# Ai00-X/ai00_server

Measured on AMD Instinct MI355X. Metric: decode tokens/sec (whole job), higher is better.
Workload: dtype u8->f16/f32acc; 1 GPU; RWKV-v6-3b int8 decode, batch=32/GPU, greedy, state+tokens resident in HBM; quant=int8, batch_per_gpu=32, parallelism=replicas x1 (no collective)

## Files before the change

### ai00_server_amd/build.py

```python
from __future__ import annotations

import os
import subprocess
import sys

HERE = os.path.dirname(os.path.abspath(__file__))
CSRC = os.path.join(HERE, "csrc")
LIB = os.path.join(HERE, "librwkv_hip.so")
SOURCES = ["rwkv_kernels.hip", "rwkv_engine.cpp", "tokenizer.cpp"]
DEPS = SOURCES + ["rwkv_kernels.h", "gemm_plan.h", "graph_cache.h", "gen_stop.h", "safetensors.hpp", "rwkv_abi.map", os.path.join("..", "..", "include", "rwkv_abi.h"),
               os.path.join("..", "..", "include", "rwkv_runtime.hpp"), os.path.join("..", "..", "include", "rwkv_scheduler.hpp"),
               os.path.join("..", "..", "include", "rwkv_router.hpp"),
               os.path.join("..", "..", "harness", "decode_loop.cpp"), os.path.join("..", "..", "harness", "serve_loop.cpp"),
               os.path.join("..", "..", "harness", "router_loop.cpp")]


def _hipcc() -> str:
    for c in (os.environ.get("HIPCC"), "/opt/rocm/bin/hipcc", "hipcc"):
        if c and (os.path.isabs(c) and os.path.exists(c) or not os.path.isabs(c)):
            return c
    return "hipcc"


STAMP = os.path.join(HERE, ".build_stamp")


def _sources_digest() -> str:
    import hashlib
    h = hashlib.sha256()
    for d in sorted(DEPS):
        with open(os.path.join(CSRC, d), "rb") as f:
            h.update(d.encode())
            h.update(f.read())
    return h.hexdigest()


def needs_build() -> bool:
    if not all(os.path.exists(p) for p in (LIB, HARNESS_BIN, SERVE_BIN, ROUTER_BIN, EMBED_BIN, STAMP)):
        return True
    return open(STAMP).read().strip() != _sources_digest()


KERNEL_PARTS = 6


def build(force: bool = False, verbose: bool = True) -> str:
    if not force and not needs_build():
        return LIB
    from concurrent.futures import ThreadPoolExecutor
    hipcc = _hipcc()
    jobs = []
    for src in SOURCES:
        stem = os.path.splitext(src)[0]
        base = [hipcc, "--offload-arch=gfx950", "-O3", "-std=c++17", "-fPIC"]
        if src.endswith(".cpp"):
            base += ["-x", "hip"]
        if src == "rwkv_kernels.hip":
            for k in range(KERNEL_PARTS):
                obj = os.path.join(CSRC, f"{stem}.p{k}.o")
                jobs.append((base + [f"-DRWKV_PART={k}", "-c", os.path.join(CSRC, src), "-o", obj], obj))
        else:
            obj = os.path.join(CSRC, stem + ".o")
            jobs.append((base + ["-c", os.path.join(CSRC, src), "-o", obj], obj))

    def run(job):
        if verbose:
            print("[build]", " ".join(job[0]), flush=True)
        subprocess.check_call(job[0])
        return job[1]

    with ThreadPoolExecutor(max_workers=min(len(jobs), os.cpu_count() or 4)) as ex:
        objs = list(ex.map(run, jobs))
    cmd = [hipcc, "--offload-arch=gfx950", "-shared", "-fPIC", "-Wl,--version-script=" + os.path.join(CSRC, "rwkv_abi.map"), "-o", LIB] + objs
    if verbose:
        print("[build]", " ".join(cmd), flush=True)
    subprocess.check_call(cmd)
    build_harness(verbose)
    with open(STAMP, "w") as f:
        f.write(_sources_digest())
    return LIB


HARNESS_SRC = os.path.join(HERE, "..", "harness", "decode_loop.cpp")
HARNESS_BIN = os.path.join(HERE, "..", "harness", "decode_loop")
SERVE_SRC = os.path.join(HERE, "..", "harness", "serve_loop.cpp")
SERVE_BIN = os.path.join(HERE, "..", "harness", "serve_loop")
ROUTER_SRC = os.path.join(HERE, "..", "harness", "router_loop.cpp")
ROUTER_BIN = os.path.join(HERE, "..", "harness", "router_loop")
EMBED_SRC = os.path.join(HERE, "..", "harness", "embed_job.cpp")
EMBED_BIN = os.path.join(HERE, "..", "harness", "embed_job")


def build_harness(verbose: bool = True) -> str:
    for src, exe in ((HARNESS_SRC, HARNESS_BIN), (SERVE_SRC, SERVE_BIN), (ROUTER_SRC, ROUTER_BIN), (EMBED_SRC, EMBED_BIN)):
        cmd = ["g++", "-O2", "-std=c++17", "-pthread", src, "-o", exe, "-L" + HERE, "-lrwkv_hip", "-Wl,-rpath," + HERE]
        if verbose:
            print("[build]", " ".join(cmd), flush=True)
        subprocess.check_call(cmd)
    return HARNESS_BIN


PROBE_DIR = os.path.join(HERE, "..", "tests", "cpp")
PROBE_SRC = os.path.join(PROBE_DIR, "gemm_probe.hip")
PROBE_BIN = os.path.join(PROBE_DIR, "gemm_probe")
PROBE_STAMP = os.path.join(PROBE_DIR, ".gemm_probe_stamp")


def compile_gemm_probe(obj: str) -> str:
    subprocess.check_call([_hipcc(), "--offload-arch=gfx950", "-O2", "-std=c++17", "-c", PROBE_SRC, "-o", obj])
    return obj


def build_gemm_probe(verbose: bool = True) -> str:
    import hashlib
    build(verbose=verbose)
    h = hashlib.sha256(_sources_digest().encode())
    for src in (PROBE_SRC, os.path.join(PROBE_DIR, "gemm_probe_plan.h")):
        with open(src, "rb") as f:
            h.update(f.read())
    if os.path.exists(PROBE_BIN) and os.path.exists(PROBE_STAMP) and open(PROBE_STAMP).read().strip() == h.hexdigest():
        return PROBE_BIN
    parts = [os.path.join(CSRC, f"rwkv_kernels.p{k}.o") for k in range(KERNEL_PARTS)]
    if not all(os.path.exists(p) for p in parts):
        build(force=True, verbose=verbose)
    obj = compile_gemm_probe(os.path.join(PROBE_DIR, "gemm_probe.o"))
    cmd = [_hipcc(), "--offload-arch=gfx950", obj] + parts + ["-o", PROBE_BIN]
    if verbose:
        print("[build]", " ".join(cmd), flush=True)
    subprocess.check_call(cmd)
    with open(PROBE_STAMP, "w") as f:
        f.write(h.hexdigest())
    return PROBE_BIN


if __name__ == "__main__":
    build(force="--force" in sys.argv)
    print(LIB)
```

### ai00_server_amd/csrc/rwkv_kernels.h

```cpp
#pragma once
#ifdef __HIP__
#include <hip/hip_runtime.h>
#else
typedef struct ihipStream_t *hipStream_t;
#ifndef __FLT16_MANT_DIG__
typedef unsigned short _Float16;
#endif
#endif
#include <stddef.h>
#include <stdint.h>

#include "gen_stop.h"

namespace rwkv {

enum WFmt : int { W_F16 = 0, W_INT8 = 1, W_NF4 = 2 };
enum Act : int { ACT_NONE = 0, ACT_TANH = 1, ACT_SIGMOID = 2, ACT_RELU2 = 3, ACT_SILU = 4, ACT_DECAY7 = 5 };
enum Post : int { POST_NONE = 0, POST_MUL = 1, POST_MIX = 2 };

struct Knobs {
    int no_ln_fuse = 0;
    int no_v6_fuse = 0;
    int no_tile = 0, tile_shape = -1;
    int no_dense = 0;
    int tile_ksplit = 1;
    int tile_xcd = -1;
    int promote = -1;
    int v6_ksp_max = 16;
    int v6_ksp_blocks = 160, v6_ksp_min_t = 192;
    static Knobs from_env();
};
const Knobs &knobs();
void use_knobs(const Knobs &k);

constexpr int TILE_ROWS = 16;
constexpr int KSTEP = 32;
constexpr int GEMM_MAX_WAVES = 10;
constexpr int GEMM_MAX_WAVES_K16 = 8;
constexpr int GEMM_MAXP = 8;
constexpr int INT8_BLOCK = 128;
constexpr int NF4_BLOCK = 64;

struct DMat {
    const void *data = nullptr;
    const void *scales = nullptr;
    int fmt = W_F16;
    int rows = 0;
    int K = 0;
    uint64_t bytes = 0;
};

struct RowMeta {
    const int *token;
    const int *slot;
    const int *prev;
    const int *last;
    int dense;
};

constexpr int LNP_MAX_T = 1;
constexpr int LNP_MAX_NP = 5;
struct LnProArgs {
    const float *x_in;
    float *x_out;
    const float *P;
    int np;
    long pstride;
    const float *lnw, *lnb;
    const float *sx;
    long sx_slot_stride;
    RowMeta rm;
    int mode;
    float *xx_out;
    int C;
};
struct ShiftCommit {
    const float *src;
    float *sx;
    long sx_slot_stride;
    RowMeta rm;
    int T, C;
};

struct GemmProb {
    const void *W;
    const void *S;
    const _Float16 *xhi;
    const _Float16 *xlo;
    int fmt, rows, K, ldx;
    int spb;
    int nw;
    int ksb;
    int Kb, nslice;
    int nblk_strip;
    int block_begin;
    int act, post;
    const float *bias;
    const float *m0, *m1;
    int ldm;
    float *out_f32;
    int ldo;
    long partial_stride;
    _Float16 *out_hi, *out_lo;
    int ldh;
};

struct GemmLaunch {
    GemmProb p[GEMM_MAXP];
    int nprob;
    int T;
    int threads;
    int lds_items;
    int single_shot;
    int tail;
    int total_blocks;
    int xcd_map;
    ShiftCommit commit;
};

size_t lnp_lds_bytes(int T, int C, bool hilo);
void launch_gemm(const GemmLaunch &L, bool hilo, hipStream_t s);
void launch_smallk(const GemmLaunch &L, bool hilo, hipStream_t s);
void launch_gemm_tile45(const GemmLaunch &L, int kind, int ntl, bool hilo, hipStream_t s);
void launch_gemm_tile(const GemmLaunch &L, int shape, bool hilo, hipStream_t s);

struct V6MixArgs {
    const void *W1;
    const void *W2[5];
    const _Float16 *zhi, *zlo;
    int ldz;
    const float *xx, *dx;
    const float *mu[5];
    _Float16 *ohi[5], *olo[5];
    int ldh, T, C, Dm;
    LnProArgs lnp;
    const float *mu_x;
    _Float16 *mg_hi = nullptr, *mg_lo = nullptr;
    float *mp = nullptr;
    int ksp = 1, ksp_min_t = 192, ksp_blocks = 160, ksp_max = 16;
};
bool v6_mix_supported(int T, int C, int Dm);
bool v6_mix_wide_supported(int T, int C, int Dm);
bool v6_mix_ln_supported(int T, int C, int Dm, bool hilo, int np);
int v6_mix_split(const V6MixArgs &a, bool hilo);
void launch_v6_mix(const V6MixArgs &a, bool hilo, hipStream_t s);


struct LnShiftArgs {
    const float *x_in;
    float *x_out;
    const float *P;
    int np;
    long pstride;
    const float *lnw, *lnb;
    float *sx;
    long sx_slot_stride;
    RowMeta rm;
    int mode;
    int nmix;
    const float *mu[6];
    _Float16 *ohi[6];
    _Float16 *olo[6];
    int ldh;
    float *xx_out, *dx_out;
    int C;
    int xcd_rows = 0;
};
void launch_ln_shift(const LnShiftArgs &a, int T, hipStream_t s);

struct EmbedArgs {
    const _Float16 *emb;
    const float *lnw, *lnb;
    const int *token;
    float *x;
    int C, V;
};
void launch_embed(const EmbedArgs &a, int T, hipStream_t s);

struct LnOutArgs {
    const float *x_in;
    const float *P;
    int np;
    long pstride;
    const float *lnw, *lnb;
    const int *out_rows;
    _Float16 *ohi, *olo;
    int ldh, C;
};
void launch_ln_out(const LnOutArgs &a, int n_out, hipStream_t s);

struct WkvArgs {
    int version;
    int H, C;
    int n_seq;
    const int *seq_slot;
    const int *seq_begin;
    const int *seq_len;
    int dense;
    float *state;
    long slot_stride;
    const float *r, *k, *v;
    const float *g;
    const float *wdec_or_decay;
    const float *u;
    const float *td;
    const _Float16 *D2;
    int Dd;
    const float *w7, *a7, *vg7;
    const float *k_k, *k_a, *r_k;
    float *v_first;
    int layer;
    const float *lnx_w, *lnx_b;
    _Float16 *yhi, *ylo;
    int ldh;
    int max_rows;
};
void launch_wkv(const WkvArgs &a, bool multi_row, hipStream_t s);

struct StatePackArgs {
    float *slab;
    float *sxa, *sxf;
    float *wkv;
    int L, C, H;
    int transposed;
    int to_slab;
    int layer_only;
};
void launch_state_pack(const StatePackArgs &a, hipStream_t s);

void launch_softmax(const float *in, float *out, int n_rows, int V, hipStream_t s);
void launch_score_rows(const float *logits, const unsigned *targets, float *out, int n_rows, int V, hipStream_t s);
struct SampleRow { float top_p; int top_k; float temperature; float uniform; int kind; float tau; };
void launch_logit_adjust(float *logits, int V, const int *rows, const int *toks, const float *vals, int n, hipStream_t s);
void launch_logit_mask(float *logits, int V, const int *rows, const unsigned char *allow, int n, hipStream_t s);
void launch_nucleus(const float *logits, int n_rows, int V, const SampleRow *sp, bool any_nucleus_typical, bool any_mirostat,
                    int *out_tok, float *out_prob, hipStream_t s);
constexpr unsigned GEN_ABSENT = 0xFFFFFFFFu;
constexpr int GEN_MAX_STOP = 8;
struct GenSlot {
    float top_p; int top_k; float temperature; float tau;
    int kind;
    float presence, frequency, decay;
    float miro_target, miro_rate;
    unsigned long long seed;
    unsigned stream, draws;
    int max_tokens, emitted, finish;
    int freeze_at;
    int has_bias, n_stop;
    unsigned stop[GEN_MAX_STOP];
// ... 52 lines not shown
```

### ai00_server_amd/csrc/rwkv_kernels.hip

```cpp
#include "gemm_plan.h"
#include <type_traits>
#include <cstdlib>
#include <algorithm>


#ifdef RWKV_PART
#define RWKV_PART_ON(k) (RWKV_PART == (k))
#else
#define RWKV_PART_ON(k) 1
#endif
#if defined(RWKV_TRACE) && defined(RWKV_PART)
#error "trace builds are single-part"
#endif

namespace rwkv {

typedef _Float16 f16x8 __attribute__((ext_vector_type(8)));
typedef _Float16 f16x4 __attribute__((ext_vector_type(4)));
typedef _Float16 f16x2 __attribute__((ext_vector_type(2)));
typedef float f32x4 __attribute__((ext_vector_type(4)));
typedef float f32x2 __attribute__((ext_vector_type(2)));
typedef unsigned int u32;
typedef unsigned int u32x4 __attribute__((ext_vector_type(4)));
typedef unsigned int u32x2 __attribute__((ext_vector_type(2)));

__device__ __forceinline__ float sigmoidf_(float x) { return 1.0f / (1.0f + expf(-x)); }

__device__ __forceinline__ float apply_act(int act, float v) {
    switch (act) {
        case ACT_TANH: return tanhf(v);
        case ACT_SIGMOID: return sigmoidf_(v);
        case ACT_RELU2: { float r = fmaxf(v, 0.0f); return r * r; }
        case ACT_SILU: return v * sigmoidf_(v);
        case ACT_DECAY7: return expf(-0.606531f * sigmoidf_(v));
        default: return v;
    }
}

__device__ __forceinline__ void apply_act4(int act, float (&v)[4]) {
    switch (act) {
        case ACT_NONE: break;
        case ACT_TANH: for (int r = 0; r < 4; ++r) v[r] = tanhf(v[r]); break;
        case ACT_SIGMOID: for (int r = 0; r < 4; ++r) v[r] = sigmoidf_(v[r]); break;
        case ACT_RELU2: for (int r = 0; r < 4; ++r) { const float q = fmaxf(v[r], 0.0f); v[r] = q * q; } break;
        case ACT_SILU: for (int r = 0; r < 4; ++r) v[r] = v[r] * sigmoidf_(v[r]); break;
        case ACT_DECAY7: for (int r = 0; r < 4; ++r) v[r] = expf(-0.606531f * sigmoidf_(v[r])); break;
        default: break;
    }
}
__device__ __forceinline__ void split_hilo(float v, _Float16 &hi, _Float16 &lo) {
    float c = fminf(fmaxf(v, -65504.0f), 65504.0f);
    hi = (_Float16)c;
    lo = (_Float16)(c - (float)hi);
}

__device__ __forceinline__ long opd_off(int t, int k, int ld) {
    return ((long)(t >> 4) * (ld >> 5) + (k >> 5)) * 512 + ((((k >> 3) & 3) << 4) + (t & 15)) * 8 + (k & 7);
}

__device__ __forceinline__ void store_operand4(_Float16 *__restrict__ hi, _Float16 *__restrict__ lo, long off, float4 o) {
    f16x4 h, l;
    _Float16 a, b;
    split_hilo(o.x, a, b); h[0] = a; l[0] = b;
    split_hilo(o.y, a, b); h[1] = a; l[1] = b;
    split_hilo(o.z, a, b); h[2] = a; l[2] = b;
    split_hilo(o.w, a, b); h[3] = a; l[3] = b;
    *(f16x4 *)(hi + off) = h;
    if (lo) *(f16x4 *)(lo + off) = l;
}

typedef __amdgpu_buffer_rsrc_t act_t;
constexpr int ACT_SC1 = 0;
__device__ __forceinline__ act_t act_buf(const void *p) {
    return __builtin_amdgcn_make_buffer_rsrc(const_cast<void *>(p), 0, -1, 0x00020000);
}
__device__ __forceinline__ float4 act_ld4(act_t b, long fidx) {
    return __builtin_bit_cast(float4, __builtin_amdgcn_raw_buffer_load_b128(b, (unsigned)(fidx * 4), 0, ACT_SC1));
}
__device__ __forceinline__ float act_ld1(act_t b, long fidx) {
    return __builtin_bit_cast(float, __builtin_amdgcn_raw_buffer_load_b32(b, (unsigned)(fidx * 4), 0, ACT_SC1));
}
__device__ __forceinline__ f16x8 act_ldh8(act_t b, long hidx) {
    return __builtin_bit_cast(f16x8, __builtin_amdgcn_raw_buffer_load_b128(b, (unsigned)(hidx * 2), 0, ACT_SC1));
}
__device__ __forceinline__ void act_st4(act_t b, long fidx, float4 v) {
    __builtin_amdgcn_raw_buffer_store_b128(__builtin_bit_cast(u32x4, v), b, (unsigned)(fidx * 4), 0, ACT_SC1);
}
__device__ __forceinline__ void act_st1(act_t b, long fidx, float v) {
    __builtin_amdgcn_raw_buffer_store_b32(__builtin_bit_cast(u32, v), b, (unsigned)(fidx * 4), 0, ACT_SC1);
}
__device__ __forceinline__ void act_sth4(act_t b, long hidx, f16x4 v) {
    __builtin_amdgcn_raw_buffer_store_b64(__builtin_bit_cast(u32x2, v), b, (unsigned)(hidx * 2), 0, ACT_SC1);
}
__device__ __forceinline__ void act_store_operand4(act_t hi, act_t lo, bool has_lo, long off, float4 o) {
    f16x4 h, l;
    _Float16 a, b;
    split_hilo(o.x, a, b); h[0] = a; l[0] = b;
    split_hilo(o.y, a, b); h[1] = a; l[1] = b;
    split_hilo(o.z, a, b); h[2] = a; l[2] = b;
    split_hilo(o.w, a, b); h[3] = a; l[3] = b;
    act_sth4(hi, off, h);
    if (has_lo) act_sth4(lo, off, l);
}

template <int CTRL>
__device__ __forceinline__ float dpp_f32(float v) {
    return __builtin_bit_cast(float, __builtin_amdgcn_update_dpp(0, __builtin_bit_cast(int, v), CTRL, 0xf, 0xf, true));
}
__device__ __forceinline__ float row_sum16(float v) {
    v += dpp_f32<0xB1>(v);
    v += dpp_f32<0x4E>(v);
    v += dpp_f32<0x124>(v);
    v += dpp_f32<0x128>(v);
    return v;
}
__device__ __forceinline__ float quad_sum(float v) {
    v += dpp_f32<0xB1>(v);
    v += dpp_f32<0x4E>(v);
    return v;
}
__device__ __forceinline__ float wave_sum(float v) {
    v = row_sum16(v);
    return (__builtin_bit_cast(float, __builtin_amdgcn_readlane(__builtin_bit_cast(int, v), 0)) +
            __builtin_bit_cast(float, __builtin_amdgcn_readlane(__builtin_bit_cast(int, v), 16))) +
           (__builtin_bit_cast(float, __builtin_amdgcn_readlane(__builtin_bit_cast(int, v), 32)) +
            __builtin_bit_cast(float, __builtin_amdgcn_readlane(__builtin_bit_cast(int, v), 48)));
}

__device__ __forceinline__ float block_sum256(float v, float *red) {
    v = wave_sum(v);
    __syncthreads();
    if ((threadIdx.x & 63) == 0) red[threadIdx.x >> 6] = v;
    __syncthreads();
    return red[0] + red[1] + red[2] + red[3];
}

template <int FMT> struct Fmt;
template <> struct Fmt<W_F16> { static constexpr int TK = 32, KS = 1, SH = 5; };
template <> struct Fmt<W_INT8> { static constexpr int TK = 64, KS = 2, SH = 6; };
template <> struct Fmt<W_NF4> { static constexpr int TK = 128, KS = 4, SH = 7; };

#ifdef RWKV_TRACE
__device__ unsigned long long g_trace[4096 * 8];
#define TRACE_PT(i) do { if ((threadIdx.x & 63) == 0 && blockIdx.x < 256) g_trace[((blockIdx.x * 16 + (threadIdx.x >> 6)) << 3) + (i)] = wall_clock64(); } while (0)
extern "C" int rwkv_debug_trace(unsigned long long *out, int n) {
    int rc = (int)hipMemcpyFromSymbol(out, HIP_SYMBOL(g_trace), (size_t)n * 8, 0, hipMemcpyDeviceToHost);
    static unsigned long long zeros[4096 * 8];
    (void)hipMemcpyToSymbol(HIP_SYMBOL(g_trace), zeros, sizeof(zeros), 0, hipMemcpyHostToDevice);
    return rc;
}
__device__ unsigned long long g_trace2[4 * 2048 * 8];
#define TRACE_K(kid, i) do { const unsigned lb_ = blockIdx.x + gridDim.x * blockIdx.y; if (threadIdx.x == 0 && lb_ < 2048) g_trace2[(((kid) * 2048 + lb_) << 3) + (i)] = wall_clock64(); } while (0)
extern "C" int rwkv_debug_trace2(unsigned long long *out) {
    int rc = (int)hipMemcpyFromSymbol(out, HIP_SYMBOL(g_trace2), sizeof(g_trace2), 0, hipMemcpyDeviceToHost);
    return rc;
}
#else
#define TRACE_PT(i) do { } while (0)
#define TRACE_K(kid, i) do { } while (0)
#endif

constexpr int RS = 8;
template <int FMT> struct WRound {
    u32x4 q[RS / Fmt<FMT>::KS];
    uint2 s;
};

__device__ __forceinline__ f16x2 as_h2(u32 v) { return __builtin_bit_cast(f16x2, v); }
__device__ __forceinline__ u32 as_u32(f16x2 v) { return __builtin_bit_cast(u32, v); }

template <int FMT, bool TAIL>
__device__ __forceinline__ void load_round(WRound<FMT> &w, const GemmProb &P, int strip, int k0, int kend, bool ok, int lane) {
    constexpr int NTILE = RS / Fmt<FMT>::KS, TK = Fmt<FMT>::TK, SH = Fmt<FMT>::SH;
    const int KT = P.K >> SH;
    const u32x4 *base = (const u32x4 *)P.W + ((long)strip * KT + (k0 >> SH)) * 64 + lane;
#pragma unroll
    for (int j = 0; j < NTILE; ++j) {
        if (!TAIL || (ok && k0 + j * TK < kend)) w.q[j] = __builtin_nontemporal_load(base + j * 64);
        else w.q[j] = (u32x4){0u, 0u, 0u, 0u};
    }
    if constexpr (FMT != W_F16) {
        const int NG = P.K >> 8;
        const uint2 *sb = (const uint2 *)P.S + ((long)strip * NG + (k0 >> 8)) * 16 + (lane & 15);
        w.s = (!TAIL || (ok && k0 < kend)) ? *sb : make_uint2(0, 0);
    } else {
        w.s = make_uint2(0, 0);
    }
}

__device__ __forceinline__ u32 dq8(u32 d, u32 sel, f16x2 a2, f16x2 b2) {
    u32 p = __builtin_amdgcn_perm(0x64646464u, d, sel);
    f16x2 h = as_h2(p) - (f16x2){(_Float16)1024.0f, (_Float16)1024.0f};
    return as_u32(__builtin_elementwise_fma(h, a2, b2));
}

static __device__ __constant__ unsigned short nf4_f16_bits[16] = {
    0xBC00, 0xB992, 0xB833, 0xB652, 0xB48D, 0xB1EA, 0xADD4, 0x0000,
    0x2D18, 0x3126, 0x33E0, 0x3568, 0x370D, 0x3880, 0x39C9, 0x3C00};

struct Nf4Lut { u32 tl[4], th[4]; };
__device__ __forceinline__ Nf4Lut make_nf4_lut() {
    Nf4Lut t;
#pragma unroll
    for (int d = 0; d < 4; ++d) {
        u32 lo = 0, hi = 0;
#pragma unroll
        for (int b = 0; b < 4; ++b) {
            u32 v = nf4_f16_bits[d * 4 + b];
            lo |= (v & 0xFF) << (8 * b);
            hi |= (v >> 8) << (8 * b);
        }
        t.tl[d] = lo; t.th[d] = hi;
    }
    return t;
}
__device__ __forceinline__ void nf4_lookup4(u32 n, const Nf4Lut &t, u32 &h01, u32 &h23) {
    u32 sel = n & 0x07070707u;
    u32 mask = ((n >> 3) & 0x01010101u) * 0xFFu;
    u32 la = __builtin_amdgcn_perm(t.tl[1], t.tl[0], sel);
    u32 lb = __builtin_amdgcn_perm(t.tl[3], t.tl[2], sel);
    u32 ha = __builtin_amdgcn_perm(t.th[1], t.th[0], sel);
    u32 hb = __builtin_amdgcn_perm(t.th[3], t.th[2], sel);
    u32 L = (la & ~mask) | (lb & mask);
    u32 Hh = (ha & ~mask) | (hb & mask);
    h01 = __builtin_amdgcn_perm(Hh, L, 0x05010400u);
    h23 = __builtin_amdgcn_perm(Hh, L, 0x07030602u);
}

template <int FMT>
__device__ __forceinline__ f16x8 frag(const WRound<FMT> &w, int ks, const Nf4Lut &lut) {
    if constexpr (FMT == W_F16) {
        return __builtin_bit_cast(f16x8, w.q[ks]);
    } else if constexpr (FMT == W_INT8) {
        const u32x4 q = w.q[ks >> 1];
        const u32 d0 = (ks & 1) ? q.z : q.x, d1 = (ks & 1) ? q.w : q.y;
        const u32 ab = (ks >> 2) ? w.s.y : w.s.x;
        const f16x2 abh = as_h2(ab);
        const f16x2 a2 = {abh[0], abh[0]}, b2 = {abh[1], abh[1]};
        u32x4 r;
        r.x = dq8(d0, 0x04010400u, a2, b2);
        r.y = dq8(d0, 0x04030402u, a2, b2);
        r.z = dq8(d1, 0x04010400u, a2, b2);
        r.w = dq8(d1, 0x04030402u, a2, b2);
        return __builtin_bit_cast(f16x8, r);
    } else {
        const u32x4 q = w.q[ks >> 2];
        const int wsel = ks & 3;
        const u32 d = wsel == 0 ? q.x : wsel == 1 ? q.y : wsel == 2 ? q.z : q.w;
        const u32 sw = (ks >> 2) ? w.s.y : w.s.x;
        const f16x2 sh = as_h2(sw);
        const _Float16 am = ((ks >> 1) & 1) ? sh[1] : sh[0];
        const f16x2 am2 = {am, am};
        u32x4 r;
        u32 a, b;
        nf4_lookup4(d & 0x0F0F0F0Fu, lut, a, b);
        r.x = as_u32(as_h2(a) * am2);
        r.y = as_u32(as_h2(b) * am2);
        nf4_lookup4((d >> 4) & 0x0F0F0F0Fu, lut, a, b);
        r.z = as_u32(as_h2(a) * am2);
        r.w = as_u32(as_h2(b) * am2);
        return __builtin_bit_cast(f16x8, r);
    }
}

constexpr int LNP_PAD = 4;
__device__ __forceinline__ float4 lnp_ld4(const float *p) { return *(const float4 *)p; }
__device__ __forceinline__ float lnp_mix1(int mode, float x, float p, float m) {
    return mode == 0 ? x * m + p * (1.0f - m) : x + (p - x) * m;
}
constexpr int LNP_PTN = 2;
struct LnCarry { int prev[LNP_MAX_T]; };
__device__ __forceinline__ void ln_prologue_load(const LnProArgs &a, int T, float *xx_l, float *pv_l, float *red,
                                                 bool publish, LnCarry &k) {
    constexpr int PTN = LNP_PTN;
    const int tid = threadIdx.x, nth = blockDim.x, lane = tid & 63, wave = tid >> 6;
    const int C = a.C, ldl = C + LNP_PAD;
    int (&prev)[LNP_MAX_T] = k.prev;
    const act_t bx = act_buf(a.x_in), bP = act_buf(a.P), bsx = act_buf(a.sx), bxo = act_buf(a.x_out);
#pragma unroll
    for (int t = 0; t < LNP_MAX_T; ++t) {
        if (t < T) {
            const int slot = a.rm.dense ? t : a.rm.slot[t];
            prev[t] = a.rm.dense ? -1 : a.rm.prev[t];
            float4 v[PTN], sxv[PTN], pp[LNP_MAX_NP][PTN];
#pragma unroll
            for (int i = 0; i < PTN; ++i) {
                const int c = (tid + i * nth) * 4;
                if (c < C) {
                    v[i] = act_ld4(bx, (long)t * C + c);
#pragma unroll
                    for (int j = 0; j < LNP_MAX_NP; ++j)
                        pp[j][i] = act_ld4(bP, (j < a.np ? j : 0) * a.pstride + (long)t * C + c);
                    sxv[i] = act_ld4(bsx, (long)slot * a.sx_slot_stride + c);
                }
            }
            float sum = 0.f;
#pragma unroll
            for (int i = 0; i < PTN; ++i) {
                const int c = (tid + i * nth) * 4;
                if (c < C) {
#pragma unroll
                    for (int j = 0; j < LNP_MAX_NP; ++j) {
                        const bool on = j < a.np;
                        v[i].x += on ? pp[j][i].x : 0.f; v[i].y += on ? pp[j][i].y : 0.f;
                        v[i].z += on ? pp[j][i].z : 0.f; v[i].w += on ? pp[j][i].w : 0.f;
                    }
                    if (publish) act_st4(bxo, (long)t * C + c, v[i]);
                    *(float4 *)(xx_l + t * ldl + c) = v[i];
                    *(float4 *)(pv_l + t * ldl + c) = sxv[i];
                    sum += (v[i].x + v[i].y) + (v[i].z + v[i].w);
                }
            }
            sum = wave_sum(sum);
            if (lane == 0) red[t * 16 + wave] = sum;
            __builtin_amdgcn_sched_barrier(0);
        }
    }
}
template <bool HILO>
__device__ __forceinline__ void ln_prologue_finish(const LnProArgs &a, int T, const float *mu, float *xx_l, float *pv_l, _Float16 *op_l,
                                                   float *red, bool publish, const LnCarry &k) {
    constexpr int PTN = LNP_PTN;
    const int tid = threadIdx.x, nth = blockDim.x, nwv = nth >> 6, lane = tid & 63, wave = tid >> 6;
    const int C = a.C, ldl = C + LNP_PAD;
    const int (&prev)[LNP_MAX_T] = k.prev;
    const act_t bxxo = act_buf(a.xx_out);
    float4 wv[PTN], bv[PTN], muv[PTN];
#pragma unroll
    for (int i = 0; i < PTN; ++i) {
        const int c = (tid + i * nth) * 4;
        if (c < C) { wv[i] = lnp_ld4(a.lnw + c); bv[i] = lnp_ld4(a.lnb + c); muv[i] = lnp_ld4(mu + c); }
    }
    __syncthreads();
    float mean[LNP_MAX_T];
#pragma unroll
    for (int t = 0; t < LNP_MAX_T; ++t) {
        mean[t] = 0.f;
        if (t < T) {
            float m = 0.f, q = 0.f;
            for (int w2 = 0; w2 < nwv; ++w2) m += red[t * 16 + w2];
            mean[t] = m / (float)C;
#pragma unroll
            for (int i = 0; i < PTN; ++i) {
                const int c = (tid + i * nth) * 4;
                if (c < C) {
                    const float4 v = *(const float4 *)(xx_l + t * ldl + c);
                    const float d0 = v.x - mean[t], d1 = v.y - mean[t], d2 = v.z - mean[t], d3 = v.w - mean[t];
                    q += (d0 * d0 + d1 * d1) + (d2 * d2 + d3 * d3);
                }
            }
            q = wave_sum(q);
            if (lane == 0) red[32 + t * 16 + wave] = q;
        }
    }
    __syncthreads();
#pragma unroll
    for (int t = 0; t < LNP_MAX_T; ++t) {
        if (t < T) {
            float m = 0.f;
            for (int w2 = 0; w2 < nwv; ++w2) m += red[32 + t * 16 + w2];
            const float rstd = 1.0f / sqrtf(m / (float)C + 1e-5f);
#pragma unroll
            for (int i = 0; i < PTN; ++i) {
                const int c = (tid + i * nth) * 4;
                if (c < C) {
                    const float4 v = *(const float4 *)(xx_l + t * ldl + c);
                    float4 o;
                    o.x = (v.x - mean[t]) * rstd * wv[i].x + bv[i].x;
                    o.y = (v.y - mean[t]) * rstd * wv[i].y + bv[i].y;
                    o.z = (v.z - mean[t]) * rstd * wv[i].z + bv[i].z;
                    o.w = (v.w - mean[t]) * rstd * wv[i].w + bv[i].w;
                    *(float4 *)(xx_l + t * ldl + c) = o;
                    if (publish) act_st4(bxxo, (long)t * C + c, o);
                }
            }
        }
    }
    __syncthreads();
    _Float16 *op_lo = op_l + (size_t)T * C;
#pragma unroll
    for (int t = 0; t < LNP_MAX_T; ++t) {
        if (t < T) {
#pragma unroll
            for (int i = 0; i < PTN; ++i) {
                const int c = (tid + i * nth) * 4;
                if (c < C) {
                    const float4 x = *(const float4 *)(xx_l + t * ldl + c);
                    const float4 pvv = prev[t] >= 0 ? *(const float4 *)(xx_l + prev[t] * ldl + c) : *(const float4 *)(pv_l + t * ldl + c);
                    const float o0 = lnp_mix1(a.mode, x.x, pvv.x, muv[i].x), o1 = lnp_mix1(a.mode, x.y, pvv.y, muv[i].y);
                    const float o2 = lnp_mix1(a.mode, x.z, pvv.z, muv[i].z), o3 = lnp_mix1(a.mode, x.w, pvv.w, muv[i].w);
                    f16x4 hh, ll;
                    _Float16 h, l;
                    split_hilo(o0, h, l); hh[0] = h; ll[0] = l;
                    split_hilo(o1, h, l); hh[1] = h; ll[1] = l;
                    split_hilo(o2, h, l); hh[2] = h; ll[2] = l;
                    split_hilo(o3, h, l); hh[3] = h; ll[3] = l;
                    const int off = ((((c >> 5) << 2) + ((c >> 3) & 3)) * T + t) * 8 + (c & 7);
                    *(f16x4 *)(op_l + off) = hh;
                    if constexpr (HILO) *(f16x4 *)(op_lo + off) = ll;
                }
            }
        }
    }
    __syncthreads();
}
__device__ __forceinline__ size_t lnp_op_off(int T, int k, int tl) { return (size_t)((k >> 3) * T + tl) * 8; }
#if RWKV_PART_ON(0)
static int knob_env(const char *name, int dflt) {
    const char *v = std::getenv(name);
    return (v && *v) ? std::atoi(v) : dflt;
}
Knobs Knobs::from_env() {
    Knobs k;
    k.no_ln_fuse = knob_env("RWKV_NO_LN_FUSE", 0); k.no_v6_fuse = knob_env("RWKV_NO_V6_FUSE", 0);
    k.no_tile = knob_env("RWKV_NO_TILE", 0); k.tile_shape = knob_env("RWKV_TILE_SHAPE", -1);
    k.no_dense = knob_env("RWKV_NO_DENSE", 0);
    k.tile_ksplit = knob_env("RWKV_TILE_KSPLIT", 1); k.tile_xcd = knob_env("RWKV_TILE_XCD", -1);
    k.promote = knob_env("RWKV_PROMOTE", -1);
    k.v6_ksp_max = knob_env("RWKV_V6_KSP_MAX", 16); k.v6_ksp_blocks = knob_env("RWKV_V6_KSP_BLOCKS", 160); k.v6_ksp_min_t = knob_env("RWKV_V6_KSP_MIN_T", 192);
    return k;
}
static thread_local Knobs t_knobs;
const Knobs &knobs() { return t_knobs; }
void use_knobs(const Knobs &k) { t_knobs = k; }

size_t lnp_lds_bytes(int T, int C, bool hilo) { return (size_t)(2 * T * (C + LNP_PAD) + 64) * 4 + (size_t)T * C * 2 * (hilo ? 2 : 1); }
#endif

__device__ __forceinline__ void shift_commit(const ShiftCommit &c) {
    for (int t = 0; t < c.T; ++t) {
        const int last = c.rm.dense ? t : c.rm.last[t];
        if (last < 0) continue;
        const act_t src = act_buf(c.src);
        float *dst = c.sx + (long)(c.rm.dense ? t : c.rm.slot[t]) * c.sx_slot_stride;
        for (int i = threadIdx.x * 4; i < c.C; i += blockDim.x * 4) *(float4 *)(dst + i) = act_ld4(src, (long)last * c.C + i);
    }
}

#if RWKV_PART_ON(0)
__device__ __forceinline__ int pin_s(int v) { v = __builtin_amdgcn_readfirstlane(v); asm volatile("" : "+s"(v)); return v; }
__device__ __forceinline__ const void *pin_p(const void *p) {
    const unsigned long long v = (unsigned long long)p;
    const unsigned lo = (unsigned)pin_s((int)(unsigned)v), hi = (unsigned)pin_s((int)(unsigned)(v >> 32));
    return (const void *)(((unsigned long long)hi << 32) | lo);
}
template <int NT, int KSW, bool HILO, bool SHOT, bool TAIL, int FMT>
__device__ __forceinline__ void gemm_body(const GemmLaunch &L, const GemmProb &P, unsigned char *smem) {
    constexpr int KW = KSW * 32, SUB = KSW / RS, RK = RS * 32;
    const int tid = threadIdx.x, lane = tid & 63;
    const int wave = __builtin_amdgcn_readfirstlane(tid >> 6);
    const int lb = (int)blockIdx.x - P.block_begin;
    const int kb = P.ksb == 1 ? 0 : lb / P.nblk_strip, sb = lb - kb * P.nblk_strip;
    const int spb = P.spb, nw = P.nw;
    const int strip0 = sb * spb;
    const int nstrip = min(spb, (P.rows >> 4) - strip0);
    const int Kb = P.Kb;
    const int kbeg = kb * Kb, kend = kbeg + Kb;
    const int nslice = P.nslice;
    f32x4 *red = (f32x4 *)smem;

    Nf4Lut lut;
    if constexpr (FMT == W_NF4) lut = make_nf4_lut();

    auto mma_round = [&](const WRound<FMT> &w, f32x4 (&acc)[NT], f32x4 (&acc2)[NT], const f16x8 (&xb)[NT][KSW],
                         const f16x8 (*xl)[HILO ? KSW : 1], int sub, int k0) {
#pragma unroll
        for (int ks = 0; ks < RS; ++ks) {
            if (!TAIL || k0 + (sub * RS + ks) * 32 < kend) {
                const f16x8 a = frag<FMT>(w, ks, lut);
#pragma unroll
                for (int nt = 0; nt < NT; ++nt) {
                    f32x4 &d = (NT == 1 && (ks & 1)) ? acc2[nt] : acc[nt];
                    d = __builtin_amdgcn_mfma_f32_16x16x32_f16(a, xb[nt][sub * RS + ks], d, 0, 0, 0);
                    if constexpr (HILO) d = __builtin_amdgcn_mfma_f32_16x16x32_f16(a, xl[nt][sub * RS + ks], d, 0, 0, 0);
                }
            }
        }
    };

    const act_t bxh = act_buf(P.xhi), bxl = act_buf(P.xlo);
    const act_t bo32 = act_buf(P.out_f32 ? P.out_f32 + (long)kb * P.partial_stride : nullptr);
    const act_t boh = act_buf(P.out_hi), bol = act_buf(P.out_lo), bm0 = act_buf(P.m0), bm1 = act_buf(P.m1);

    constexpr int MAXR = (NT == 4 || (NT == 2 && HILO)) ? 2 : (FMT == W_F16 ? 2 : ((NT == 2 || HILO) ? 3 : 4));
    WRound<FMT> cur, nxt, w[SHOT ? MAXR : 1];
    constexpr int RD = (!SHOT && FMT != W_F16) ? ((NT >= 2 || HILO) ? 2 : 4) : 1;
    WRound<FMT> ring[RD];
    auto issue_w = [&](int k0, int nsub, int nround, bool ringed) {
        if constexpr (SHOT) {
#pragma unroll
            for (int r = 0; r < MAXR; ++r) {
                const int s = r / SUB, sub = r % SUB;
                if (s < nstrip && sub < nsub) load_round<FMT, TAIL>(w[r], P, strip0 + s, k0 + sub * RK, kend, true, lane);
            }
        } else if (ringed) {
#pragma unroll
            for (int j = 0; j < RD; ++j)
                if (j < nround) load_round<FMT, TAIL>(ring[j], P, strip0 + j / SUB, k0 + (j % SUB) * RK, kend, true, lane);
        } else {
            load_round<FMT, TAIL>(cur, P, strip0, k0, kend, true, lane);
        }
    };

    TRACE_PT(0);
    for (int t0 = 0; t0 < L.T; t0 += NT * 16) {
        for (int sl = wave; sl < nslice && wave < nw; sl += nw) {
            const int k0 = kbeg + sl * KW;
            const int nsub = TAIL ? SUB : min(SUB, (kend - k0) / RK);
            const int nround = nstrip * nsub;
            TRACE_PT(6);
            f16x8 xb[NT][KSW], xl[HILO ? NT : 1][HILO ? KSW : 1];
            const bool ringed = RD > 1 && nsub == SUB;
            auto load_x = [&]() {
#pragma unroll
                for (int nt = 0; nt < NT; ++nt) {
                    const int tile = min((t0 >> 4) + nt, (L.T - 1) >> 4);
                    const int tl = min(lane & 15, L.T - 1 - tile * 16);
                    const long xo = ((long)tile * (P.ldx >> 5) + (k0 >> 5)) * 512 + ((lane >> 4) * 16 + tl) * 8;
#pragma unroll
                    for (int sub = 0; sub < SUB; ++sub) {
                        if (TAIL || sub < nsub) {
#pragma unroll
                            for (int k8 = 0; k8 < RS; ++k8) {
                                const int ks = sub * RS + k8;
                                const bool in = !TAIL || (k0 + ks * 32 < kend);
                                xb[nt][ks] = in ? act_ldh8(bxh, xo + ks * 512) : (f16x8){0, 0, 0, 0, 0, 0, 0, 0};
                                if constexpr (HILO) xl[nt][ks] = in ? act_ldh8(bxl, xo + ks * 512) : (f16x8){0, 0, 0, 0, 0, 0, 0, 0};
                            }
                        } else {
#pragma unroll
                            for (int k8 = 0; k8 < RS; ++k8) {
                                xb[nt][sub * RS + k8] = (f16x8){0, 0, 0, 0, 0, 0, 0, 0};
                                if constexpr (HILO) xl[nt][sub * RS + k8] = (f16x8){0, 0, 0, 0, 0, 0, 0, 0};
                            }
                        }
                    }
                }
            };
            load_x();
            TRACE_PT(7);
            issue_w(k0, nsub, nround, ringed);
#ifdef RWKV_TRACE
            TRACE_PT(1);
#if RWKV_TRACE >= 2
            asm volatile("s_waitcnt vmcnt(0)" ::: "memory");
            TRACE_PT(5);
#endif
#endif
            f32x4 acc[NT], acc2[NT];
            auto park = [&](int s) {
                f32x4 *slot = red + ((s * nw + wave) * NT) * 64 + lane;
#pragma unroll
                for (int nt = 0; nt < NT; ++nt) {
                    const f32x4 v = acc[nt] + acc2[nt];
                    if (sl == wave) slot[nt * 64] = v; else slot[nt * 64] += v;
                }
            };
            if constexpr (SHOT) {
#pragma unroll
                for (int r = 0; r < MAXR; ++r) {
                    const int s = r / SUB, sub = r % SUB;
                    if (s < nstrip) {
                        if (sub == 0) {
#pragma unroll
                            for (int nt = 0; nt < NT; ++nt) acc[nt] = acc2[nt] = (f32x4){0.f, 0.f, 0.f, 0.f};
                        }
                        if (sub < nsub) mma_round(w[r], acc, acc2, xb, xl, sub, k0);
                        if (sub == SUB - 1) park(s);
                    }
                }
            } else if (ringed) {
                for (int r0 = 0; r0 < nround; r0 += RD) {
#pragma unroll
                    for (int j = 0; j < RD; ++j) {
                        const int r = r0 + j, s = r / SUB;
                        constexpr int SUBM = SUB - 1;
                        const int sub = j & SUBM;
                        if (r < nround) {
                            if (sub == 0) {
#pragma unroll
                                for (int nt = 0; nt < NT; ++nt) acc[nt] = acc2[nt] = (f32x4){0.f, 0.f, 0.f, 0.f};
                            }
                            mma_round(ring[j], acc, acc2, xb, xl, sub, k0);
                            if (r + RD < nround)
                                load_round<FMT, TAIL>(ring[j], P, strip0 + (r + RD) / SUB, k0 + sub * RK, kend, true, lane);
                            if (sub == SUB - 1) park(s);
                        }
                    }
                }
            } else {
                for (int s = 0; s < nstrip; ++s) {
#pragma unroll
                    for (int sub = 0; sub < SUB; ++sub) {
                        if (sub < nsub) {
                            const bool more_sub = sub + 1 < nsub;
                            if (more_sub || s + 1 < nstrip)
                                load_round<FMT, TAIL>(nxt, P, strip0 + (more_sub ? s : s + 1), k0 + (more_sub ? sub + 1 : 0) * RK, kend, true, lane);
                            if (sub == 0) {
#pragma unroll
                                for (int nt = 0; nt < NT; ++nt) acc[nt] = acc2[nt] = (f32x4){0.f, 0.f, 0.f, 0.f};
                            }
                            mma_round(cur, acc, acc2, xb, xl, sub, k0);
                            cur = nxt;
                        }
                    }
                    park(s);
                }
            }
            (void)nround;
        }
        TRACE_PT(2);
        const int e_act = pin_s(P.act), e_post = pin_s(P.post), e_ldm = pin_s(P.ldm), e_ldo = pin_s(P.ldo), e_ldh = pin_s(P.ldh);
        const float *e_bias = (const float *)pin_p(P.bias);
        const bool e_f32 = pin_s(P.out_f32 != nullptr) != 0, e_hi = pin_s(P.out_hi != nullptr) != 0, e_lo = pin_s(P.out_lo != nullptr) != 0;
        const int nwaves = blockDim.x >> 6, nitem = nstrip * NT;
        float4 pb = make_float4(0.f, 0.f, 0.f, 0.f), pm0 = pb, pm1 = pb;
        auto prefetch = [&](int item) {
            const int s = item / NT, nt = item - s * NT;
            const int row0 = (strip0 + s) * 16 + (lane >> 4) * 4;
            const int t = t0 + nt * 16 + (lane & 15);
            if (t < L.T) {
                if (e_bias) pb = *(const float4 *)(e_bias + row0);
                if (e_post != POST_NONE) pm0 = act_ld4(bm0, (long)t * e_ldm + row0);
                if (e_post == POST_MIX) pm1 = act_ld4(bm1, (long)t * e_ldm + row0);
            }
        };
        if (wave < nitem) prefetch(wave);
        __syncthreads();
        TRACE_PT(3);
        for (int item = wave; item < nitem; item += nwaves) {
            if (item != wave) prefetch(item);
            const int s = item / NT, nt = item - s * NT;
            const f32x4 *rp = red + ((s * nw) * NT + nt) * 64 + lane;
            f32x4 v4 = rp[0];
            for (int w2 = 1; w2 < nw; w2 += 3) {
                const f32x4 zero = {0.f, 0.f, 0.f, 0.f};
                const f32x4 pa = rp[w2 * NT * 64];
                const f32x4 pb2 = w2 + 1 < nw ? rp[(w2 + 1) * NT * 64] : zero;
                const f32x4 pc = w2 + 2 < nw ? rp[(w2 + 2) * NT * 64] : zero;
                v4 += pa; v4 += pb2; v4 += pc;
            }
            const int row0 = (strip0 + s) * 16 + (lane >> 4) * 4;
            const int t = t0 + nt * 16 + (lane & 15);
            if (t < L.T) {
                float v[4] = {v4[0], v4[1], v4[2], v4[3]};
                if (e_bias) { v[0] += pb.x; v[1] += pb.y; v[2] += pb.z; v[3] += pb.w; }
                apply_act4(e_act, v);
                if (e_post == POST_MUL) {
                    v[0] *= pm0.x; v[1] *= pm0.y; v[2] *= pm0.z; v[3] *= pm0.w;
                } else if (e_post == POST_MIX) {
                    v[0] = pm0.x + pm1.x * v[0]; v[1] = pm0.y + pm1.y * v[1]; v[2] = pm0.z + pm1.z * v[2]; v[3] = pm0.w + pm1.w * v[3];
                }
                if (e_f32) act_st4(bo32, (long)t * e_ldo + row0, make_float4(v[0], v[1], v[2], v[3]));
                if (e_hi) act_store_operand4(boh, bol, e_lo, opd_off(t, row0, e_ldh), make_float4(v[0], v[1], v[2], v[3]));
            }
        }
        if (t0 + NT * 16 < L.T) __syncthreads();
    }
    TRACE_PT(4);
}

template <int NT, int KSW, bool HILO, bool SHOT, bool TAIL>
__global__ __launch_bounds__(((NT == 4 || (NT == 2 && HILO)) ? GEMM_MAX_WAVES_K16 : GEMM_MAX_WAVES) * 64) void gemm_kernel(const GemmLaunch L) {
    extern __shared__ __attribute__((aligned(16))) unsigned char smem[];
    if ((int)blockIdx.x >= L.total_blocks) {
        shift_commit(L.commit);
        return;
    }
    int pi = 0;
    for (int i = 1; i < L.nprob; ++i)
        if ((int)blockIdx.x >= L.p[i].block_begin) pi = i;
    const GemmProb &P = L.p[pi];
    if (P.fmt == W_F16) gemm_body<NT, KSW, HILO, SHOT, TAIL, W_F16>(L, P, smem);
    else if (P.fmt == W_INT8) gemm_body<NT, KSW, HILO, SHOT, false, W_INT8>(L, P, smem);
    else gemm_body<NT, KSW, HILO, SHOT, false, W_NF4>(L, P, smem);
}

void launch_gemm(const GemmLaunch &L, bool hilo, hipStream_t s) {
    int NT, KSW;
    gemm_variant(L.T, hilo, NT, KSW);
    const size_t lds = (size_t)L.lds_items * NT * 64 * 16;
    dim3 grid(L.total_blocks + (L.commit.src ? 1 : 0)), block(L.threads);
    static bool attr_done[16] = {false};
    int dev = 0;
    (void)hipGetDevice(&dev);
#define GEMM_V3(X, sh, tl) X(1, 8, true, sh, tl) X(2, 8, true, sh, tl) X(2, 8, false, sh, tl) X(1, 8, false, sh, tl) X(4, 8, false, sh, tl)
#define GEMM_VARIANTS(X) GEMM_V3(X, true, true) GEMM_V3(X, true, false) GEMM_V3(X, false, true) GEMM_V3(X, false, false)
    if (!attr_done[dev & 15]) {
        const int cap = 160 * 1024;
#define SET_ATTR(a, b, c, d, e) (void)hipFuncSetAttribute((const void *)gemm_kernel<a, b, c, d, e>, hipFuncAttributeMaxDynamicSharedMemorySize, cap);
        GEMM_VARIANTS(SET_ATTR)
#undef SET_ATTR
        attr_done[dev & 15] = true;
    }
    const bool shot = L.single_shot != 0, tail = L.tail != 0;
#define LAUNCH(a, b, c, d, e) if (NT == a && KSW == b && hilo == c && shot == d && tail == e) hipLaunchKernelGGL((gemm_kernel<a, b, c, d, e>), grid, block, lds, s, L);
    GEMM_VARIANTS(LAUNCH)
#undef LAUNCH
#undef GEMM_VARIANTS
#undef GEMM_V3
}

#endif


#if RWKV_PART_ON(1)
template <int NT, bool HILO, int DS, bool LNP, bool WIDE = false, bool P1ONLY = false>
__global__ __launch_bounds__(512) void v6_mix_kernel(const V6MixArgs a) {
    extern __shared__ __attribute__((aligned(16))) unsigned char smem[];
    const int tid = threadIdx.x, lane = tid & 63;
    const int wave = __builtin_amdgcn_readfirstlane(tid >> 6);
    const int c = blockIdx.y;
    const int sg = blockIdx.x;
    const int C = a.C, Dm = a.Dm, T = a.T;
    const int tz = blockIdx.z;
    const int t0 = tz * NT * 16;
    const int KT1 = C >> 5;
    const int ksp = P1ONLY ? a.ksp : 1, kq = P1ONLY ? (int)blockIdx.x : 0;
    const int kst = (KT1 >> 3) / ksp;
    const int kw0 = (kq * 8 + wave) * kst;
    f32x4 *red = (f32x4 *)smem;
    const int mstride = Dm + 8;
    _Float16 *m_hi = (_Float16 *)(smem + (size_t)8 * 4 * NT * 64 * 16);
    _Float16 *m_lo = m_hi + NT * 16 * mstride;

    TRACE_K(0, 0);
    const int strip = sg * 8 + wave;
    const int strip_c = min(strip, (C >> 4) - 1);
    const int row0 = strip_c * 16 + (lane >> 4) * 4;
    u32x4 w2t[DS / 2];
    float4 xxv[NT], dxv[NT];
    float4 mu = make_float4(0.f, 0.f, 0.f, 0.f);
    if constexpr (!WIDE) {
#pragma unroll
        for (int ks = 0; ks < DS / 2; ++ks) w2t[ks] = ((const u32x4 *)a.W2[c])[((long)strip_c * (DS / 2) + ks) * 64 + lane];
        mu = *(const float4 *)(a.mu[c] + row0);
    }
    const act_t bxx = act_buf(a.xx), bdx = act_buf(a.dx), bzh = act_buf(a.zhi), bzl = act_buf(a.zlo);
    const act_t boh = act_buf(a.ohi[c]), bol = act_buf(a.olo[c]);
    float *xx_l = (float *)(m_lo + NT * 16 * mstride);
    const int ldl = C + LNP_PAD;
    float *pv_l = xx_l + LNP_MAX_T * ldl, *lred = pv_l + LNP_MAX_T * ldl;
    _Float16 *z_l = (_Float16 *)(lred + 64);
    const u32x4 *w1 = (const u32x4 *)a.W1;
    constexpr int KB = DS == 2 ? ((HILO && NT == 2) ? 5 : 10) : 4;
    u32x4 wt[KB][DS];
    auto load_wt = [&](int k0) {
#pragma unroll
        for (int j = 0; j < KB; ++j) {
            if (k0 + j < kst) {
                const int kt = kw0 + k0 + j;
#pragma unroll
                for (int d = 0; d < DS; ++d) wt[j][d] = w1[((long)(c * DS + d) * KT1 + kt) * 64 + lane];
            }
        }
    };
    if constexpr (LNP) {
        LnCarry carry;
        const bool pub = blockIdx.x == 0 && blockIdx.y == 0;
        load_wt(0);
        ln_prologue_load(a.lnp, T, xx_l, pv_l, lred, pub, carry);
        ln_prologue_finish<HILO>(a.lnp, T, a.mu_x, xx_l, pv_l, z_l, lred, pub, carry);
#pragma unroll
        for (int nt = 0; nt < NT; ++nt) {
            const int t = min(nt * 16 + (lane & 15), T - 1);
            const float4 x = *(const float4 *)(xx_l + t * ldl + row0);
            const float4 pr = carry.prev[t < LNP_MAX_T ? t : 0] >= 0 ? *(const float4 *)(xx_l + carry.prev[t < LNP_MAX_T ? t : 0] * ldl + row0)
                                                                      : *(const float4 *)(pv_l + t * ldl + row0);
            xxv[nt] = x;
            dxv[nt] = make_float4(pr.x - x.x, pr.y - x.y, pr.z - x.z, pr.w - x.w);
        }
    } else if constexpr (!WIDE) {
#pragma unroll
        for (int nt = 0; nt < NT; ++nt) {
            int t = t0 + nt * 16 + (lane & 15);
            t = t < T ? t : T - 1;
            xxv[nt] = act_ld4(bxx, (long)t * C + row0);
            dxv[nt] = act_ld4(bdx, (long)t * C + row0);
        }
    }
    f32x4 acc[DS][NT];
#pragma unroll
    for (int d = 0; d < DS; ++d)
#pragma unroll
        for (int nt = 0; nt < NT; ++nt) acc[d][nt] = (f32x4){0.f, 0.f, 0.f, 0.f};
    for (int k0 = 0; k0 < kst; k0 += KB) {
        f16x8 zb[KB][NT], zl[HILO ? KB : 1][HILO ? NT : 1];
        if (!LNP || k0 > 0) load_wt(k0);
#pragma unroll
        for (int j = 0; j < KB; ++j) {
            if (k0 + j < kst) {
                const int kt = kw0 + k0 + j;
#pragma unroll
                for (int nt = 0; nt < NT; ++nt) {
                    const int tile = min((t0 >> 4) + nt, (T - 1) >> 4);
                    const int tl = min(lane & 15, T - 1 - tile * 16);
                    if constexpr (LNP) {
                        zb[j][nt] = *(const f16x8 *)(z_l + lnp_op_off(T, kt * 32 + (lane >> 4) * 8, tl));
                        if constexpr (HILO) zl[j][nt] = *(const f16x8 *)(z_l + (size_t)T * C + lnp_op_off(T, kt * 32 + (lane >> 4) * 8, tl));
                    } else {
                        const long zo = ((long)tile * (a.ldz >> 5) + kt) * 512 + ((lane >> 4) * 16 + tl) * 8;
                        zb[j][nt] = act_ldh8(bzh, zo);
                        if constexpr (HILO) zl[j][nt] = act_ldh8(bzl, zo);
                    }
                }
            }
        }
#pragma unroll
        for (int j = 0; j < KB; ++j) {
            if (k0 + j < kst) {
#pragma unroll
                for (int d = 0; d < DS; ++d) {
                    const f16x8 af = __builtin_bit_cast(f16x8, wt[j][d]);
#pragma unroll
                    for (int nt = 0; nt < NT; ++nt) {
                        acc[d][nt] = __builtin_amdgcn_mfma_f32_16x16x32_f16(af, zb[j][nt], acc[d][nt], 0, 0, 0);
                        if constexpr (HILO) acc[d][nt] = __builtin_amdgcn_mfma_f32_16x16x32_f16(af, zl[j][nt], acc[d][nt], 0, 0, 0);
                    }
                }
            }
        }
    }
#pragma unroll
    for (int d = 0; d < DS; ++d)
#pragma unroll
        for (int nt = 0; nt < NT; ++nt) red[((wave * 4 + d) * NT + nt) * 64 + lane] = acc[d][nt];
    TRACE_K(0, 1);
    __syncthreads();
    TRACE_K(0, 2);
    for (int item = wave; item < DS * NT; item += 8) {
        const int d = item / NT, nt = item - d * NT;
        f32x4 v = red[((0 * 4 + d) * NT + nt) * 64 + lane];
        for (int w2 = 1; w2 < 8; ++w2) v += red[((w2 * 4 + d) * NT + nt) * 64 + lane];
        const int t = nt * 16 + (lane & 15);
        if constexpr (P1ONLY) {
            if (ksp > 1) {
                const long po = (((long)kq * 5 + c) * ((long)gridDim.z * NT * 16) + t0 + t) * Dm + d * 16 + (lane >> 4) * 4;
                *(f32x4 *)(a.mp + po) = v;
                continue;
            }
        }
        f16x4 hh, ll;
#pragma unroll
        for (int r = 0; r < 4; ++r) { _Float16 x, y; split_hilo(tanhf(v[r]), x, y); hh[r] = x; ll[r] = y; }
        if constexpr (P1ONLY) {
            const long mo = (((long)c * gridDim.z + tz) * (NT * 16) + t) * Dm + d * 16 + (lane >> 4) * 4;
            *(f16x4 *)(a.mg_hi + mo) = hh;
            if constexpr (HILO) *(f16x4 *)(a.mg_lo + mo) = ll;
        } else {
// ... 2462 lines not shown
```

Before: 14130 tokens/s.

## Deal leftover K-slices across idle waves in hilo NT=2 GEMM

When the K-slice count does not divide evenly among waves, the remainder slices are no longer walked by a few waves while others idle. Each leftover slice is split into two jobs, one per 16-column tile, and handed to otherwise idle waves. Their partial sums go into extra LDS reduction slots that the epilogue folds in. This aims to cut load imbalance in the split-K reduction, at the cost of more LDS, extra weight loads without the nontemporal hint, and extra reduction reads.

```diff
diff --git a/ai00_server_amd/build.py b/ai00_server_amd/build.py
--- a/ai00_server_amd/build.py
+++ b/ai00_server_amd/build.py
@@ -8,7 +8,7 @@
 CSRC = os.path.join(HERE, "csrc")
 LIB = os.path.join(HERE, "librwkv_hip.so")
 SOURCES = ["rwkv_kernels.hip", "rwkv_engine.cpp", "tokenizer.cpp"]
-DEPS = SOURCES + ["rwkv_kernels.h", "gemm_plan.h", "graph_cache.h", "gen_stop.h", "safetensors.hpp", "rwkv_abi.map", os.path.join("..", "..", "include", "rwkv_abi.h"),
+DEPS = SOURCES + ["rwkv_kernels.h", "gemm_plan.h", "gemm_deal.h", "graph_cache.h", "gen_stop.h", "safetensors.hpp", "rwkv_abi.map", os.path.join("..", "..", "include", "rwkv_abi.h"),
                os.path.join("..", "..", "include", "rwkv_runtime.hpp"), os.path.join("..", "..", "include", "rwkv_scheduler.hpp"),
                os.path.join("..", "..", "include", "rwkv_router.hpp"),
                os.path.join("..", "..", "harness", "decode_loop.cpp"), os.path.join("..", "..", "harness", "serve_loop.cpp"),
diff --git a/ai00_server_amd/csrc/gemm_deal.h b/ai00_server_amd/csrc/gemm_deal.h
--- /dev/null
+++ b/ai00_server_amd/csrc/gemm_deal.h
@@ -0,0 +1,24 @@
+#pragma once
+
+#if defined(__HIPCC__)
+#define RWKV_DEAL_FN __host__ __device__ inline
+#else
+#define RWKV_DEAL_FN inline
+#endif
+
+namespace rwkv {
+
+RWKV_DEAL_FN int overflow_slices(int nslice, int nw) {
+    const int r = nslice % nw;
+    return (r > 0 && 2 * r <= nw) ? r : 0;
+}
+
+struct OverflowJob { int slice, tile, col; };
+
+RWKV_DEAL_FN OverflowJob overflow_job(int nslice, int nw, int ovr, int wave) {
+    const int j = wave;
+    if (ovr <= 0 || j < 0 || j >= 2 * ovr || j >= nw) return {-1, 0, 0};
+    return {nslice - ovr + (j >> 1), j & 1, j >> 1};
+}
+
+}
diff --git a/ai00_server_amd/csrc/rwkv_kernels.h b/ai00_server_amd/csrc/rwkv_kernels.h
--- a/ai00_server_amd/csrc/rwkv_kernels.h
+++ b/ai00_server_amd/csrc/rwkv_kernels.h
@@ -26,6 +26,7 @@
     int tile_ksplit = 1;
     int tile_xcd = -1;
     int promote = -1;
+    int no_hilo_deal = 0;
     int v6_ksp_max = 16;
     int v6_ksp_blocks = 160, v6_ksp_min_t = 192;
     static Knobs from_env();
@@ -95,6 +96,7 @@
     int nblk_strip;
     int block_begin;
     int act, post;
+    int ovr;
     const float *bias;
     const float *m0, *m1;
     int ldm;
diff --git a/ai00_server_amd/csrc/rwkv_kernels.hip b/ai00_server_amd/csrc/rwkv_kernels.hip
--- a/ai00_server_amd/csrc/rwkv_kernels.hip
+++ b/ai00_server_amd/csrc/rwkv_kernels.hip
@@ -1,4 +1,5 @@
 #include "gemm_plan.h"
+#include "gemm_deal.h"
 #include <type_traits>
 #include <cstdlib>
 #include <algorithm>
@@ -169,14 +170,14 @@
 __device__ __forceinline__ f16x2 as_h2(u32 v) { return __builtin_bit_cast(f16x2, v); }
 __device__ __forceinline__ u32 as_u32(f16x2 v) { return __builtin_bit_cast(u32, v); }
 
-template <int FMT, bool TAIL>
+template <int FMT, bool TAIL, bool STREAM = true>
 __device__ __forceinline__ void load_round(WRound<FMT> &w, const GemmProb &P, int strip, int k0, int kend, bool ok, int lane) {
     constexpr int NTILE = RS / Fmt<FMT>::KS, TK = Fmt<FMT>::TK, SH = Fmt<FMT>::SH;
     const int KT = P.K >> SH;
     const u32x4 *base = (const u32x4 *)P.W + ((long)strip * KT + (k0 >> SH)) * 64 + lane;
 #pragma unroll
     for (int j = 0; j < NTILE; ++j) {
-        if (!TAIL || (ok && k0 + j * TK < kend)) w.q[j] = __builtin_nontemporal_load(base + j * 64);
+        if (!TAIL || (ok && k0 + j * TK < kend)) w.q[j] = STREAM ? __builtin_nontemporal_load(base + j * 64) : base[j * 64];
         else w.q[j] = (u32x4){0u, 0u, 0u, 0u};
     }
     if constexpr (FMT != W_F16) {
@@ -416,7 +417,7 @@
     k.no_tile = knob_env("RWKV_NO_TILE", 0); k.tile_shape = knob_env("RWKV_TILE_SHAPE", -1);
     k.no_dense = knob_env("RWKV_NO_DENSE", 0);
     k.tile_ksplit = knob_env("RWKV_TILE_KSPLIT", 1); k.tile_xcd = knob_env("RWKV_TILE_XCD", -1);
-    k.promote = knob_env("RWKV_PROMOTE", -1);
+    k.promote = knob_env("RWKV_PROMOTE", -1); k.no_hilo_deal = knob_env("RWKV_NO_HILO_DEAL", 0);
     k.v6_ksp_max = knob_env("RWKV_V6_KSP_MAX", 16); k.v6_ksp_blocks = knob_env("RWKV_V6_KSP_BLOCKS", 160); k.v6_ksp_min_t = knob_env("RWKV_V6_KSP_MIN_T", 192);
     return k;
 }
@@ -457,6 +458,9 @@
     const int Kb = P.Kb;
     const int kbeg = kb * Kb, kend = kbeg + Kb;
     const int nslice = P.nslice;
+    constexpr bool DEAL = NT == 2 && HILO;
+    const int ovr = DEAL ? P.ovr : 0;
+    const int nwalk = nslice - ovr, nwc = nw + ovr;
     f32x4 *red = (f32x4 *)smem;
 
     Nf4Lut lut;
@@ -504,7 +508,7 @@
 
     TRACE_PT(0);
     for (int t0 = 0; t0 < L.T; t0 += NT * 16) {
-        for (int sl = wave; sl < nslice && wave < nw; sl += nw) {
+        for (int sl = wave; sl < nwalk && wave < nw; sl += nw) {
             const int k0 = kbeg + sl * KW;
             const int nsub = TAIL ? SUB : min(SUB, (kend - k0) / RK);
             const int nround = nstrip * nsub;
@@ -549,7 +553,7 @@
 #endif
             f32x4 acc[NT], acc2[NT];
             auto park = [&](int s) {
-                f32x4 *slot = red + ((s * nw + wave) * NT) * 64 + lane;
+                f32x4 *slot = red + ((s * nwc + wave) * NT) * 64 + lane;
 #pragma unroll
                 for (int nt = 0; nt < NT; ++nt) {
                     const f32x4 v = acc[nt] + acc2[nt];
@@ -608,6 +612,45 @@
                 }
             }
             (void)nround;
+        }
+        if constexpr (DEAL) {
+            const OverflowJob jb = overflow_job(nslice, nw, ovr, wave);
+            if (jb.slice >= 0) {
+                static_assert(!DEAL || KSW == RS, "a job's round is a whole strip");
+                const int k0 = kbeg + jb.slice * KW;
+                TRACE_PT(6);
+                f16x8 xh[KSW], xo[KSW];
+                {
+                    const int tile = min((t0 >> 4) + jb.tile, (L.T - 1) >> 4);
+                    const int tl = min(lane & 15, L.T - 1 - tile * 16);
+                    const long xoff = ((long)tile * (P.ldx >> 5) + (k0 >> 5)) * 512 + ((lane >> 4) * 16 + tl) * 8;
+#pragma unroll
+                    for (int ks = 0; ks < KSW; ++ks) {
+                        const bool in = !TAIL || (k0 + ks * 32 < kend);
+                        xh[ks] = in ? act_ldh8(bxh, xoff + ks * 512) : (f16x8){0, 0, 0, 0, 0, 0, 0, 0};
+                        xo[ks] = in ? act_ldh8(bxl, xoff + ks * 512) : (f16x8){0, 0, 0, 0, 0, 0, 0, 0};
+                    }
+                }
+                TRACE_PT(7);
+                WRound<FMT> &jc = SHOT ? w[0] : cur, &jn = SHOT ? w[SHOT ? MAXR - 1 : 0] : nxt;
+                load_round<FMT, TAIL, false>(jc, P, strip0, k0, kend, true, lane);
+                TRACE_PT(1);
+                for (int s = 0; s < nstrip; ++s) {
+                    if (s + 1 < nstrip) load_round<FMT, TAIL, false>(jn, P, strip0 + s + 1, k0, kend, true, lane);
+                    f32x4 d = {0.f, 0.f, 0.f, 0.f};
+#pragma unroll
+                    for (int ks = 0; ks < RS; ++ks) {
+                        if (!TAIL || k0 + ks * 32 < kend) {
+                            const f16x8 a = frag<FMT>(jc, ks, lut);
+                            d = __builtin_amdgcn_mfma_f32_16x16x32_f16(a, xh[ks], d, 0, 0, 0);
+                            d = __builtin_amdgcn_mfma_f32_16x16x32_f16(a, xo[ks], d, 0, 0, 0);
+                        }
+                    }
+                    const f32x4 zero = {0.f, 0.f, 0.f, 0.f};
+                    red[((s * nwc + nw + jb.col) * NT + jb.tile) * 64 + lane] = d + zero;
+                    jc = jn;
+                }
+            }
         }
         TRACE_PT(2);
         const int e_act = pin_s(P.act), e_post = pin_s(P.post), e_ldm = pin_s(P.ldm), e_ldo = pin_s(P.ldo), e_ldh = pin_s(P.ldh);
@@ -631,13 +674,19 @@
         for (int item = wave; item < nitem; item += nwaves) {
             if (item != wave) prefetch(item);
             const int s = item / NT, nt = item - s * NT;
-            const f32x4 *rp = red + ((s * nw) * NT + nt) * 64 + lane;
+            const f32x4 *rp = red + ((s * nwc) * NT + nt) * 64 + lane;
             f32x4 v4 = rp[0];
+            if constexpr (DEAL) { if (ovr > 0) v4 += rp[nw * NT * 64]; }
             for (int w2 = 1; w2 < nw; w2 += 3) {
                 const f32x4 zero = {0.f, 0.f, 0.f, 0.f};
-                const f32x4 pa = rp[w2 * NT * 64];
-                const f32x4 pb2 = w2 + 1 < nw ? rp[(w2 + 1) * NT * 64] : zero;
-                const f32x4 pc = w2 + 2 < nw ? rp[(w2 + 2) * NT * 64] : zero;
+                f32x4 pa = rp[w2 * NT * 64];
+                f32x4 pb2 = w2 + 1 < nw ? rp[(w2 + 1) * NT * 64] : zero;
+                f32x4 pc = w2 + 2 < nw ? rp[(w2 + 2) * NT * 64] : zero;
+                if constexpr (DEAL) {
+                    if (w2 < ovr) pa += rp[(nw + w2) * NT * 64];
+                    if (w2 + 1 < ovr) pb2 += rp[(nw + w2 + 1) * NT * 64];
+                    if (w2 + 2 < ovr) pc += rp[(nw + w2 + 2) * NT * 64];
+                }
                 v4 += pa; v4 += pb2; v4 += pc;
             }
             const int row0 = (strip0 + s) * 16 + (lane >> 4) * 4;
@@ -679,7 +728,17 @@
 void launch_gemm(const GemmLaunch &L, bool hilo, hipStream_t s) {
     int NT, KSW;
     gemm_variant(L.T, hilo, NT, KSW);
-    const size_t lds = (size_t)L.lds_items * NT * 64 * 16;
+    GemmLaunch Ld = L;
+    int items = L.lds_items;
+    if (hilo && NT == 2 && !knobs().no_hilo_deal) {
+        int it = items;
+        for (int i = 0; i < L.nprob; ++i) it = std::max(it, L.p[i].spb * (L.p[i].nw + overflow_slices(L.p[i].nslice, L.p[i].nw)));
+        if ((size_t)it * NT * 64 * 16 <= (size_t)160 * 1024) {
+            items = it;
+            for (int i = 0; i < L.nprob; ++i) Ld.p[i].ovr = overflow_slices(L.p[i].nslice, L.p[i].nw);
+        }
+    }
+    const size_t lds = (size_t)items * NT * 64 * 16;
     dim3 grid(L.total_blocks + (L.commit.src ? 1 : 0)), block(L.threads);
     static bool attr_done[16] = {false};
     int dev = 0;
@@ -694,7 +753,7 @@
         attr_done[dev & 15] = true;
     }
     const bool shot = L.single_shot != 0, tail = L.tail != 0;
-#define LAUNCH(a, b, c, d, e) if (NT == a && KSW == b && hilo == c && shot == d && tail == e) hipLaunchKernelGGL((gemm_kernel<a, b, c, d, e>), grid, block, lds, s, L);
+#define LAUNCH(a, b, c, d, e) if (NT == a && KSW == b && hilo == c && shot == d && tail == e) hipLaunchKernelGGL((gemm_kernel<a, b, c, d, e>), grid, block, lds, s, Ld);
     GEMM_VARIANTS(LAUNCH)
 #undef LAUNCH
 #undef GEMM_VARIANTS
```

New measurement: 13270 tokens/s. 0.939x the previous value.
